# guy3540/Acoustic_Locating_VQ-VAE

Hardware: AMD Instinct MI355X
Metric: spectrograms/sec (train step), speech VQ-VAE default config (higher is better)
Workload: dtype x3mx_hb

## Files before the change

### acoustic_locating_vq-vae_amd/csrc/alvq_common.h

```cpp
#pragma once
#include <hip/hip_runtime.h>
#include <stdint.h>
#include <stdio.h>

#include "../../include/alvq.h"

namespace alvq {

void set_error(const char* fmt, ...);

enum Option { OPT_WIDE_MIN_TILES, OPT_FX_ROWS, OPT_FX_NARROW, OPT_FX_EPI, OPT_CONV_V2, OPT_CONV_K3, OPT_WGRAD_V3, OPT_VQ_REG, OPT_PHAT_LDS, OPT_COUNT };
long option(int id);

inline int check_launch(const char* what) {
  hipError_t e = hipGetLastError();
  if (e != hipSuccess) {
    set_error("%s: %s", what, hipGetErrorString(e));
    return (int)e;
  }
  return ALVQ_OK;
}

#define ALVQ_REQUIRE(cond, code, ...)  \
  do {                                 \
    if (!(cond)) {                     \
      alvq::set_error(__VA_ARGS__);    \
      return (code);                   \
    }                                  \
  } while (0)

struct DeviceOnce {
  bool done[64] = {};
  bool need() {
    int d = 0;
    if (hipGetDevice(&d) != hipSuccess || d < 0 || d >= 64) return true;
    if (done[d]) return false;
    done[d] = true;
    return true;
  }
};

constexpr int kWave = 64;
constexpr int kNumXcd = 8;

__device__ __forceinline__ int xcd_remap(int id, int n) {
  const int q = n / kNumXcd, r = n % kNumXcd;
  const int xcd = id % kNumXcd, local = id / kNumXcd;
  const int base = xcd < r ? xcd * (q + 1) : r * (q + 1) + (xcd - r) * q;
  return base + local;
}

typedef float f32x4 __attribute__((ext_vector_type(4)));
typedef float f32x16 __attribute__((ext_vector_type(16)));
typedef short bf16x8 __attribute__((ext_vector_type(8)));
typedef short bf16x4 __attribute__((ext_vector_type(4)));

int* fx_range_flag_ptr();
int* fx_range_sticky_ptr();

}

#include "block_reduce.h"
```

### acoustic_locating_vq-vae_amd/csrc/api.hip

```cpp
#include <stdarg.h>
#include <stdlib.h>
#include <string.h>

#include <atomic>

#include "alvq_common.h"

namespace alvq {
static thread_local char g_err[512] = "";
void set_error(const char* fmt, ...) {
  va_list ap;
  va_start(ap, fmt);
  vsnprintf(g_err, sizeof(g_err), fmt, ap);
  va_end(ap);
}

struct OptionSpec { const char* name; const char* env; long def; };
static const OptionSpec kSpecs[OPT_COUNT] = {
    {"wide_min_tiles", "ALVQ_WIDE_MIN_TILES", 192},
    {"fx_rows", "ALVQ_FX_ROWS", 0},
    {"fx_narrow", "ALVQ_FX_NARROW", 1},
    {"fx_epi", "ALVQ_FX_EPI", 1},
    {"conv_v2", "ALVQ_CONV_V2", 1},
    {"conv_k3", "ALVQ_CONV_K3", 1},
    {"wgrad_v3", "ALVQ_WGRAD_V3", 3},
    {"vq_reg", "ALVQ_VQ_REG", 1},
    {"phat_lds", "ALVQ_PHAT_LDS", 1},
};
static std::atomic<long> g_opt[OPT_COUNT];
static std::atomic<int> g_opt_ready{0};
static void options_init() {
  if (g_opt_ready.load(std::memory_order_acquire)) return;
  for (int i = 0; i < OPT_COUNT; ++i) {
    const char* e = getenv(kSpecs[i].env);
    g_opt[i].store(e ? atol(e) : kSpecs[i].def, std::memory_order_relaxed);
  }
  g_opt_ready.store(1, std::memory_order_release);
}
long option(int id) {
  options_init();
  return g_opt[id].load(std::memory_order_relaxed);
}
}

extern "C" const char* alvq_version(void) { return "alvq 0.4.0 (gfx950)"; }
extern "C" const char* alvq_last_error(void) { return alvq::g_err; }

extern "C" int alvq_set_option(const char* name, int64_t value) {
  ALVQ_REQUIRE(name, ALVQ_EINVAL, "alvq_set_option: null name");
  alvq::options_init();
  for (int i = 0; i < alvq::OPT_COUNT; ++i)
    if (!strcmp(name, alvq::kSpecs[i].name)) {
      alvq::g_opt[i].store((long)value, std::memory_order_relaxed);
      return ALVQ_OK;
    }
  alvq::set_error("alvq_set_option: unknown option '%s'", name);
  return ALVQ_EINVAL;
}

extern "C" int64_t alvq_get_option(const char* name) {
  if (name) {
    alvq::options_init();
    for (int i = 0; i < alvq::OPT_COUNT; ++i)
      if (!strcmp(name, alvq::kSpecs[i].name)) return alvq::g_opt[i].load(std::memory_order_relaxed);
  }
  alvq::set_error("alvq_get_option: unknown option '%s'", name ? name : "(null)");
  return INT64_MIN;
}
```

### acoustic_locating_vq-vae_amd/csrc/conv1d_bf16x3.hip

```cpp
#include <stdlib.h>

#include "alvq_common.h"
#include "bf16_common.h"
#include "conv_tile.h"
#include "nlc_host.h"
#include "wgrad_bias_reduce.h"
#include "wgrad_reduce.h"
#include "wgrad_tile.h"

namespace alvq {

struct ConvX3Args {
  ConvBArgs b;
  long x_plane, wp_plane, y_plane;
};

__device__ __forceinline__ void split2(float v, u16& hi, u16& lo) {
  hi = f2bf(v);
  lo = f2bf(v - bf2f(hi));
}

__device__ __forceinline__ void split_pack8(const float (&v)[8], u32x4& hi, u32x4& lo) {
#pragma unroll
  for (int e = 0; e < 4; ++e) {
    hi[e] = f2bf_pk(v[2 * e], v[2 * e + 1]);
    lo[e] = f2bf_pk(v[2 * e] - __uint_as_float(hi[e] << 16), v[2 * e + 1] - __uint_as_float(hi[e] & 0xffff0000u));
  }
}

template <int NNI>
__device__ __forceinline__ void wave_epilogue_x3(const ConvX3Args& ax, const f32x4 (&acc)[8][NNI], int m0, int r0, int li,
                                                 int kq, int wm0, int wn0) {
  const ConvBArgs& a = ax.b;
  const int Lp1 = a.L + 1, ndata = a.B * Lp1;
  const int mb0 = m0 + wm0 + (kq & 1) * 16 + (kq >> 1) * 8;
  const long pl = ax.y_plane;
#pragma unroll
  for (int ni = 0; ni < NNI; ++ni) {
    const int row = r0 + wn0 + ni * 16 + li;
    int b, l;
    const bool ok = row_valid(row, Lp1, ndata, &b, &l);
    const bool gaps = !__all(ok);
    const long o0 = (long)row * a.Mop + mb0;
    u16x8 s1h[4], s1l[4], mk[4];
#pragma unroll
    for (int mp = 0; mp < 8; mp += 2) {
      if (m0 + wm0 + mp * 16 >= a.Mop) continue;
      if (a.skip1) {
        s1h[mp / 2] = *(const u16x8*)(a.skip1 + o0 + mp * 16);
        s1l[mp / 2] = *(const u16x8*)(a.skip1 + pl + o0 + mp * 16);
      }
      if (a.mask) mk[mp / 2] = *(const u16x8*)(a.mask + o0 + mp * 16);
    }
    __builtin_amdgcn_sched_barrier(0);
#pragma unroll
    for (int mp = 0; mp < 8; mp += 2) {
      if (m0 + wm0 + mp * 16 >= a.Mop) continue;
      const long o = o0 + mp * 16;
      const int mb = mb0 + mp * 16;
      float v[8];
#pragma unroll
      for (int e = 0; e < 4; ++e) {
        const u32x2 r = __builtin_amdgcn_permlane16_swap(__float_as_uint(acc[mp][ni][e]), __float_as_uint(acc[mp + 1][ni][e]),
                                                         false, false);
        v[e] = __uint_as_float(r[0]);
        v[e + 4] = __uint_as_float(r[1]);
      }
      if (a.bias) {
        if (m0 + wm0 + mp * 16 + 32 <= a.M) {
          const f32x4 b0 = *(const f32x4*)(a.bias + mb), b1 = *(const f32x4*)(a.bias + mb + 4);
#pragma unroll
          for (int e = 0; e < 4; ++e) {
            v[e] += b0[e];
            v[4 + e] += b1[e];
          }
        } else {
#pragma unroll
          for (int e = 0; e < 8; ++e) v[e] += (mb + e < a.M) ? a.bias[mb + e] : 0.f;
        }
      }
      if (a.skip1) {
#pragma unroll
        for (int e = 0; e < 8; ++e) v[e] += bf2f(s1h[mp / 2][e]) + bf2f(s1l[mp / 2][e]);
      }
      if (a.skip2) {
        const u16x8 sh = *(const u16x8*)(a.skip2 + o), sl = *(const u16x8*)(a.skip2 + pl + o);
#pragma unroll
        for (int e = 0; e < 8; ++e) v[e] += bf2f(sh[e]) + bf2f(sl[e]);
      }
      if (a.relu & 1) {
#pragma unroll
        for (int e = 0; e < 8; ++e) v[e] = fmaxf(v[e], 0.f);
      }
      if (a.mask) {
#pragma unroll
        for (int e = 0; e < 8; ++e) v[e] = bf2f(mk[mp / 2][e]) > 0.f ? v[e] : 0.f;
      }
      u32x4 hi, lo;
      split_pack8(v, hi, lo);
      if (gaps) {
#pragma unroll
        for (int e = 0; e < 4; ++e) {
          hi[e] = ok ? hi[e] : 0u;
          lo[e] = ok ? lo[e] : 0u;
        }
      }
      *(u32x4*)(a.y + o) = hi;
      *(u32x4*)(a.y + pl + o) = lo;
      if (a.y2) {
        const u16x8 ph = *(const u16x8*)(a.post + o), pq = *(const u16x8*)(a.post + pl + o);
#pragma unroll
        for (int e = 0; e < 8; ++e) v[e] += bf2f(ph[e]) + bf2f(pq[e]);
        split_pack8(v, hi, lo);
        if (gaps) {
#pragma unroll
          for (int e = 0; e < 4; ++e) {
            hi[e] = ok ? hi[e] : 0u;
            lo[e] = ok ? lo[e] : 0u;
          }
        }
        *(u32x4*)(a.y2 + o) = hi;
        *(u32x4*)(a.y2 + pl + o) = lo;
      }
    }
  }
}

template <int NNI, int OPS>
__device__ __forceinline__ void wave_epilogue_x3_ordered(const ConvX3Args& ax, f32x4 (&acc)[8][NNI], int m0, int r0, int li,
                                                         int kq, int wm0, int wn0) {
  const ConvBArgs& a = ax.b;
  const int Lp1 = a.L + 1, ndata = a.B * Lp1;
  const int mb0 = m0 + wm0 + (kq & 1) * 16 + (kq >> 1) * 8;
  const long pl = ax.y_plane;
  const long o00 = (long)(r0 + wn0 + li) * a.Mop + mb0, oblk = (long)16 * a.Mop;
  u16x8 s1h[4], s1l[4];
  auto request = [&](int ni) {
#pragma unroll
    for (int p = 0; p < 4; ++p) {
      s1h[p] = *(const u16x8*)(a.skip1 + o00 + ni * oblk + p * 32);
      s1l[p] = *(const u16x8*)(a.skip1 + pl + o00 + ni * oblk + p * 32);
    }
  };
  if (OPS == 1) request(0);
  if (OPS == 2) {
#pragma unroll
    for (int mi = 0; mi < 8; ++mi) {
      const int c0 = m0 + wm0 + mi * 16 + kq * 4;
      f32x4 bv;
      if (m0 + wm0 + (mi & ~1) * 16 + 32 <= a.M) {
        bv = *(const f32x4*)(a.bias + c0);
      } else {
#pragma unroll
        for (int e = 0; e < 4; ++e) bv[e] = (c0 + e < a.M) ? a.bias[c0 + e] : 0.f;
      }
#pragma unroll
      for (int ni = 0; ni < NNI; ++ni)
#pragma unroll
        for (int e = 0; e < 4; ++e) acc[mi][ni][e] += bv[e];
    }
  }
  __builtin_amdgcn_sched_barrier(0);
#pragma unroll
  for (int ni = 0; ni < NNI; ++ni) {
    int b, l;
    const bool ok = row_valid(r0 + wn0 + ni * 16 + li, Lp1, ndata, &b, &l);
    const bool gaps = !__all(ok);
    u32x4 hi[4], lo[4];
#pragma unroll
    for (int p = 0; p < 4; ++p) {
      float v[8];
#pragma unroll
      for (int e = 0; e < 4; ++e) {
        const u32x2 r = __builtin_amdgcn_permlane16_swap(__float_as_uint(acc[2 * p][ni][e]), __float_as_uint(acc[2 * p + 1][ni][e]),
                                                         false, false);
        v[e] = __uint_as_float(r[0]);
        v[e + 4] = __uint_as_float(r[1]);
      }
      if (OPS == 1) {
#pragma unroll
        for (int e = 0; e < 8; ++e) v[e] += bf2f(s1h[p][e]) + bf2f(s1l[p][e]);
      }
      if (a.relu & 1) {
#pragma unroll
        for (int e = 0; e < 8; ++e) v[e] = fmaxf(v[e], 0.f);
      }
      split_pack8(v, hi[p], lo[p]);
      if (gaps) {
#pragma unroll
        for (int e = 0; e < 4; ++e) {
          hi[p][e] = ok ? hi[p][e] : 0u;
          lo[p][e] = ok ? lo[p][e] : 0u;
        }
      }
    }
    __builtin_amdgcn_sched_barrier(0);
    if (OPS == 1 && ni + 1 < NNI) request(ni + 1);
    __builtin_amdgcn_sched_barrier(0);
#pragma unroll
    for (int p = 0; p < 4; ++p) {
      *(u32x4*)(a.y + o00 + ni * oblk + p * 32) = hi[p];
      *(u32x4*)(a.y + pl + o00 + ni * oblk + p * 32) = lo[p];
    }
  }
}


template <int OUT, int KW, int NNI = 4>
__global__ __launch_bounds__(512, 2) void conv1d_bf16x3_kernel(ConvX3Args ax) {
  static_assert(NNI == 4 || NNI == 2 || NNI == 1, "4, 2 or 1 row fragments per wave");
  typedef ConvRings G;
  constexpr int MT = NNI == 4 ? G::M : 128;
  constexpr int RT = NNI == 1 ? 128 : G::R;
  const ConvBArgs& a = ax.b;
  extern __shared__ __attribute__((aligned(16))) unsigned char lds[];
  const int tid = threadIdx.x, lane = tid & 63;
  const int wave = __builtin_amdgcn_readfirstlane(tid >> 6);
  const int li = lane & 15, kq = lane >> 4;
  const int wm0 = NNI == 4 ? (wave >> 2) * 128 : 0, wn0 = NNI == 4 ? (wave & 3) * 64 : wave * 16 * NNI;

  const ConvTileOrigin o = conv_tile_origin<MT, RT>(a);
  const int m0 = o.m0, r0 = o.r0;
  const int Cp = a.Cp;
  const int srow = slab64_lane(lane).row;
  const unsigned lane_off = slab64_lane_off(lane, Cp);
  const long tap_w = (long)a.Mp128 * Cp * 2;
  const long row16 = (long)Cp * 32;
  const long wpl = ax.wp_plane * 2, xpl = ax.x_plane * 2;
  const char* const wb = (const char*)(a.wp + ((long)m0 + wave * 32) * Cp);
  const char* const xb = (const char*)(a.x + ((long)r0 - (KW - 1) / 2 + wave * 32) * Cp);
  const ConvRingStager<KW, MT, RT, false> st(wave, srow, lane_off, tap_w, row16, wpl, xpl, wb, xb);

  const int loffA = slab64_frag16(li, kq, 0);
  int loffB[KW];
#pragma unroll
  for (int t = 0; t < KW; ++t) loffB[t] = slab64_frag16(li, kq, t);
  const unsigned char* const abase = lds + wm0 * 64 + loffA;
  const unsigned char* const bbase = lds + G::XBASE + wn0 * 64;
  bf16x8_t fa0[8], fa1[8], fb0[NNI], fb1[NNI];
#define X3_RDA(DST, HALF, WS, PLANE)                                                               \
  {                                                                                                \
    const unsigned char* pa_ = abase + (WS) * G::WSTAGE + (PLANE) * G::SLAB;                       \
    _Pragma("unroll") for (int mi = (HALF) * 4; mi < (HALF) * 4 + 4; ++mi) DST[mi] = *(const bf16x8_t*)(pa_ + mi * 1024); \
  }
#define X3_RDB(DST, XS, TAP, PLANE)                                                                \
  {                                                                                                \
    const unsigned char* pb_ = bbase + (XS) * G::XSTAGE + (PLANE) * G::XSLAB + loffB[TAP];         \
    _Pragma("unroll") for (int ni = 0; ni < NNI; ++ni) DST[ni] = *(const bf16x8_t*)(pb_ + ni * 1024); \
  }

  f32x4 acc[8][NNI];
#pragma unroll
  for (int i = 0; i < 8; ++i)
#pragma unroll
    for (int j = 0; j < NNI; ++j) acc[i][j] = f32x4{0.f, 0.f, 0.f, 0.f};
#define X3_MM(A, B, HALF)                                                                          \
  _Pragma("unroll") for (int mi = (HALF) * 4; mi < (HALF) * 4 + 4; ++mi)                           \
  _Pragma("unroll") for (int ni = 0; ni < NNI; ++ni)                                               \
      asm("v_mfma_f32_16x16x32_bf16 %0, %1, %2, %0" : "+v"(acc[mi][ni]) : "v"(A[mi]), "v"(B[ni]));
#define X3_SB __builtin_amdgcn_sched_barrier(0);

  const int nch = Cp / G::K;
  const int n = nch * KW;
  const bool early = wave < 4;

  st.prologue(lds, n, nch);
  X3_RDA(fa0, 0, 0, 0)
  X3_RDA(fa0, 1, 0, 0)
  X3_RDB(fb0, 0, 0, 0)

#define X3_TILE(WS, XS, TAP, NWS, NXS, NTAP, BX, BY, DMA_)                                         \
  X3_MM(fa0, BX, 0) X3_SB X3_RDB(BY, XS, TAP, 1) X3_SB                                             \
  X3_MM(fa0, BX, 1) X3_SB X3_RDA(fa1, 0, WS, 1) X3_SB                                              \
  X3_MM(fa0, BY, 0) X3_SB X3_RDA(fa1, 1, WS, 1) X3_SB                                              \
  X3_MM(fa0, BY, 1) X3_SB                                                                          \
  asm volatile("s_waitcnt vmcnt(0) lgkmcnt(0)" ::: "memory");                                      \
  __builtin_amdgcn_s_barrier();                                                                    \
  if (early) { DMA_ }                                                                              \
  X3_MM(fa1, BX, 0) X3_SB X3_RDA(fa0, 0, NWS, 0) X3_RDB(BY, NXS, NTAP, 0) X3_SB                    \
  if (!early) { DMA_ }                                                                             \
  X3_MM(fa1, BX, 1) X3_SB X3_RDA(fa0, 1, NWS, 0) X3_SB

  if (KW == 3) {
    for (int c = 0; c < nch; c += 2) {
      const int t = 3 * c;
      X3_TILE(0, 0, 0, 1, 0, 1, fb0, fb1, if (t + 2 < n) st.issueW(lds, t + 2); if (c + 1 < nch) st.issueX(lds, c + 1, 0);)
      X3_TILE(1, 0, 1, 0, 0, 2, fb1, fb0, if (t + 3 < n) st.issueW(lds, t + 3); if (c + 1 < nch) st.issueX(lds, c + 1, 1);)
      X3_TILE(0, 0, 2, 1, 1, 0, fb0, fb1, if (t + 4 < n) st.issueW(lds, t + 4);)
      X3_TILE(1, 1, 0, 0, 1, 1, fb1, fb0, if (t + 5 < n) st.issueW(lds, t + 5); if (c + 2 < nch) st.issueX(lds, c + 2, 0);)
      X3_TILE(0, 1, 1, 1, 1, 2, fb0, fb1, if (t + 6 < n) st.issueW(lds, t + 6); if (c + 2 < nch) st.issueX(lds, c + 2, 1);)
      X3_TILE(1, 1, 2, 0, 0, 0, fb1, fb0, if (t + 7 < n) st.issueW(lds, t + 7);)
    }
  } else {
    for (int t = 0; t < n; t += 2) {
      X3_TILE(0, 0, 0, 1, 1, 0, fb0, fb1, if (t + 2 < n) { st.issueW(lds, t + 2); st.issueX(lds, t + 2, 0); st.issueX(lds, t + 2, 1); })
      X3_TILE(1, 1, 0, 0, 0, 0, fb1, fb0, if (t + 3 < n) { st.issueW(lds, t + 3); st.issueX(lds, t + 3, 0); st.issueX(lds, t + 3, 1); })
    }
  }
#undef X3_TILE
#undef X3_SB
#undef X3_MM
#undef X3_RDB
#undef X3_RDA
  asm volatile("s_nop 15\n\ts_nop 15" ::: "memory");

  if constexpr (OUT == 0) {
    const bool plain = !a.skip2 && !a.mask && !a.y2 && m0 + wm0 + 128 <= a.Mop;
    if (plain && a.skip1 && !a.bias) wave_epilogue_x3_ordered<NNI, 1>(ax, acc, m0, r0, li, kq, wm0, wn0);
    else if (plain && a.bias && !a.skip1) wave_epilogue_x3_ordered<NNI, 2>(ax, acc, m0, r0, li, kq, wm0, wn0);
    else wave_epilogue_x3(ax, acc, m0, r0, li, kq, wm0, wn0);
    return;
  }
  __syncthreads();
  conv_store_ncl<false, MT, RT>(a, lds, m0, r0, tid, nullptr, [&](float* Cs, int slab) {
    if ((wn0 >> 6) == slab) store_frags16<C_SLAB_STRIDE>(Cs, acc, li, kq, wm0, wn0 & 63);
  });
}

struct WgradX3Args {
  const u16* dy[WGRAD_MAXSEG];
  const u16* x[WGRAD_MAXSEG];
  int nseg;
  float* partial;
  float* bias_partial;
  long dy_plane, x_plane;
  int Mp, Cp, M, C;
  int mtiles, ctiles, splits, chunks_per_split, total_rows;
};

template <int KW, int NCF>
__global__ __launch_bounds__(512, 2) void conv1d_wgrad_bf16x3_kernel(WgradX3Args a) {
  constexpr int MT = 128, CT = 4 * NCF * 16;
  typedef WgradSlabs<KW, MT, CT, 2> Slabs;
  constexpr int YRB = Slabs::YRB, XRB = Slabs::XRB, YBYTES = Slabs::YBYTES, XBYTES = Slabs::XBYTES;
  extern __shared__ __attribute__((aligned(16))) unsigned char lds[];

  const int tid = threadIdx.x, lane = tid & 63;
  const int wave = __builtin_amdgcn_readfirstlane(tid >> 6);
  const int wm0 = (wave >> 2) * 64, wc0 = (wave & 3) * NCF * 16;
  const WgradWork w = wgrad_work<MT, CT>(a);
  const int n = w.n;
  WgradStager<WgradX3Args, KW, MT, CT, 2, LdsDmaAsm> st(a, wave, lane, w);

  int ybase, xbase[KW], yseg[4], xseg[NCF], xline[NCF];
  wgrad_frag16_bases<KW, NCF, YRB, XRB>(lane, wm0, wc0, ybase, xbase, yseg, xseg, xline);

  f32x4 acc[KW][4][NCF];
#pragma unroll
  for (int t = 0; t < KW; ++t)
#pragma unroll
    for (int i = 0; i < 4; ++i)
#pragma unroll
      for (int j = 0; j < NCF; ++j) acc[t][i][j] = f32x4{0.f, 0.f, 0.f, 0.f};
  const bool do_bias = a.bias_partial != nullptr && w.c0 == 0 && (wave & 3) == 0;
  f32x4 accb[4];
#pragma unroll
  for (int i = 0; i < 4; ++i) accb[i] = f32x4{0.f, 0.f, 0.f, 0.f};
  typedef short s16x8_t __attribute__((ext_vector_type(8)));
  const s16x8_t ones_raw = {0x3F80, 0x3F80, 0x3F80, 0x3F80, 0x3F80, 0x3F80, 0x3F80, 0x3F80};
  bf16x8_t ones = __builtin_bit_cast(bf16x8_t, ones_raw);
  asm volatile("" : "+v"(ones));

  bf16x8_t ah[4], al[4], b0[KW][NCF], b1[KW][NCF];
#define WX_RDA(DST, STAGE, PLANE, MI) \
  DST[MI] = wgrad_tr16_pair<bf16x8_t>(lds + ((STAGE) * STAGE_B + (PLANE) * YBYTES + (ybase ^ yseg[MI])), YRB);
#define WX_RDB(DST, STAGE, PLANE, TP, CF)                                                                                      \
  DST[TP][CF] = wgrad_tr16_pair<bf16x8_t>(                                                                                     \
      lds + ((STAGE) * STAGE_B + 2 * YBYTES + (PLANE) * XBYTES + ((xbase[TP] ^ xseg[CF]) + xline[CF])), XRB);
#define WX_MM(A, B, MI)                                                                                    \
  _Pragma("unroll") for (int tp = 0; tp < KW; ++tp)                                                        \
  _Pragma("unroll") for (int cf = 0; cf < NCF; ++cf)                                                       \
      asm("v_mfma_f32_16x16x32_bf16 %0, %1, %2, %0" : "+v"(acc[tp][MI][cf]) : "v"(A[MI]), "v"(B[tp][cf]));
#define WX_BIAS_ON(A, MI) asm("v_mfma_f32_16x16x32_bf16 %0, %1, %2, %0" : "+v"(accb[MI]) : "v"(A[MI]), "v"(ones));
#define WX_BIAS_OFF(A, MI)
#define WX_SB __builtin_amdgcn_sched_barrier(0);
  constexpr int STAGE_B = Slabs::STAGE;

#define WX_TILE(S, BX, BY, MORE, WX_BIAS)                                                                         \
                                                 \
  WX_MM(ah, BX, 0) WX_BIAS(ah, 0) WX_SB                                                                    \
  _Pragma("unroll") for (int tp = 0; tp < KW; ++tp) _Pragma("unroll") for (int cf = 0; cf < NCF; ++cf) WX_RDB(BY, S, 1, tp, cf) \
  WX_SB WX_MM(ah, BX, 1) WX_BIAS(ah, 1) WX_SB                                                              \
  WX_RDA(al, S, 1, 0) WX_RDA(al, S, 1, 1) WX_RDA(al, S, 1, 2) WX_RDA(al, S, 1, 3)                          \
  WX_SB WX_MM(ah, BX, 2) WX_BIAS(ah, 2) WX_MM(ah, BX, 3) WX_BIAS(ah, 3) WX_SB                              \
                                                                                       \
  WX_MM(ah, BY, 0) WX_MM(ah, BY, 1) WX_MM(ah, BY, 2) WX_MM(ah, BY, 3) WX_SB                                \
  asm volatile("s_waitcnt vmcnt(0) lgkmcnt(0)" ::: "memory");                                              \
  __builtin_amdgcn_s_barrier();                                                                            \
     \
  if (MORE) st.issue(lds, S);                                                                              \
  WX_MM(al, BX, 0) WX_BIAS(al, 0) WX_SB                                                                    \
  WX_RDA(ah, (S) ^ 1, 0, 0) WX_RDA(ah, (S) ^ 1, 0, 1) WX_RDA(ah, (S) ^ 1, 0, 2) WX_RDA(ah, (S) ^ 1, 0, 3)  \
  WX_SB WX_MM(al, BX, 1) WX_BIAS(al, 1) WX_SB                                                              \
  _Pragma("unroll") for (int tp = 0; tp < KW; ++tp) _Pragma("unroll") for (int cf = 0; cf < NCF; ++cf) WX_RDB(BY, (S) ^ 1, 0, tp, cf) \
  WX_SB WX_MM(al, BX, 2) WX_BIAS(al, 2) WX_MM(al, BX, 3) WX_BIAS(al, 3) WX_SB

  if (n > 0) {
    st.issue(lds, 0);
    if (n > 1) st.issue(lds, 1);
    st.wait_keep(n > 1 ? 1 : 0);
    __builtin_amdgcn_s_barrier();
    WX_RDA(ah, 0, 0, 0) WX_RDA(ah, 0, 0, 1) WX_RDA(ah, 0, 0, 2) WX_RDA(ah, 0, 0, 3)
#pragma unroll
    for (int tp = 0; tp < KW; ++tp)
#pragma unroll
      for (int cf = 0; cf < NCF; ++cf) WX_RDB(b0, 0, 0, tp, cf)
    if (do_bias) {
      for (int t = 0; t < n; t += 2) {
        WX_TILE(0, b0, b1, t + 2 < n, WX_BIAS_ON)
        WX_TILE(1, b1, b0, t + 3 < n, WX_BIAS_ON)
      }
    } else {
      for (int t = 0; t < n; t += 2) {
        WX_TILE(0, b0, b1, t + 2 < n, WX_BIAS_OFF)
        WX_TILE(1, b1, b0, t + 3 < n, WX_BIAS_OFF)
      }
    }
    asm volatile("s_nop 15\n\ts_nop 15" ::: "memory");
  }
#undef WX_TILE
#undef WX_SB
#undef WX_BIAS_ON
#undef WX_BIAS_OFF
#undef WX_MM
#undef WX_RDB
#undef WX_RDA

  wgrad_store16<KW, NCF>(a, w, lane, wm0, wc0, acc, do_bias, accb);
}

__global__ __launch_bounds__(256) void ncl_to_nlc_x3_kernel(const float* x, u16* y, long plane, int B, int C, int L, int Cp,
                                                            int rows_total) {
  __shared__ float tile[32][33];
  const int ct = Cp / 32;
  const int r0 = (blockIdx.x / ct) * 32, c0 = (blockIdx.x % ct) * 32;
  const int tx = threadIdx.x & 31, ty = threadIdx.x >> 5;
  const int Lp1 = L + 1, ndata = B * Lp1;
#pragma unroll
  for (int i = 0; i < 4; ++i) {
    const int c = c0 + ty + 8 * i, row = r0 + tx;
    int b, l;
    const bool ok = row_valid(row, Lp1, ndata, &b, &l) && c < C;
    tile[ty + 8 * i][tx] = ok ? x[((long)b * C + c) * L + l] : 0.f;
  }
  __syncthreads();
#pragma unroll
  for (int i = 0; i < 4; ++i) {
    const int row = r0 + ty + 8 * i, c = c0 + tx;
    if (row < rows_total) {
      u16 hi, lo;
      split2(tile[tx][ty + 8 * i], hi, lo);
      y[(long)row * Cp + c] = hi;
      y[plane + (long)row * Cp + c] = lo;
    }
  }
}

__global__ __launch_bounds__(256) void nlc_to_ncl_x3_kernel(const u16* x, long plane, float* y, int B, int C, int L, int Cp,
                                                            int rows_total) {
  __shared__ float tile[32][33];
  const int ct = Cp / 32;
  const int r0 = (blockIdx.x / ct) * 32, c0 = (blockIdx.x % ct) * 32;
  const int tx = threadIdx.x & 31, ty = threadIdx.x >> 5;
  const int Lp1 = L + 1, ndata = B * Lp1;
#pragma unroll
  for (int i = 0; i < 4; ++i) {
    const int row = r0 + ty + 8 * i, c = c0 + tx;
    tile[ty + 8 * i][tx] = row < rows_total ? bf2f(x[(long)row * Cp + c]) + bf2f(x[plane + (long)row * Cp + c]) : 0.f;
  }
  __syncthreads();
#pragma unroll
  for (int i = 0; i < 4; ++i) {
    const int c = c0 + ty + 8 * i, row = r0 + tx;
    int b, l;
    if (row_valid(row, Lp1, ndata, &b, &l) && c < C) y[((long)b * C + c) * L + l] = tile[tx][ty + 8 * i];
  }
}

__global__ __launch_bounds__(256) void relu_mask_x3_kernel(const u16* dy, const u16* t, u16* out, long plane8, long n8) {
  for (long e = (long)blockIdx.x * 256 + threadIdx.x; e < n8; e += (long)gridDim.x * 256) {
    const u16x8 dh = ((const u16x8*)dy)[e], dl = ((const u16x8*)dy)[plane8 + e], m = ((const u16x8*)t)[e];
    u16x8 oh, ol;
#pragma unroll
    for (int i = 0; i < 8; ++i) {
      const bool keep = bf2f(m[i]) > 0.f;
      oh[i] = keep ? dh[i] : (u16)0;
      ol[i] = keep ? dl[i] : (u16)0;
    }
    ((u16x8*)out)[e] = oh;
    ((u16x8*)out)[plane8 + e] = ol;
  }
}

template <int KW, int NCF>
static constexpr int wgrad_x3_lds() {
  return 2 * WgradSlabs<KW, 128, 4 * NCF * 16, 2>::STAGE;
}

static WgradTile wgrad_x3_tile(int KW) { return {128, KW == 3 ? 128 : 256}; }

constexpr int X3_BIAS_SPLITS = 64;

}

using namespace alvq;

extern "C" int64_t alvq_nlc_plane_bytes(int B, int L, int C) {
  return (B <= 0 || L <= 0 || C <= 0) ? -1 : nlc_plane_elems(B, L, C) * 2;
}

extern "C" int alvq_pack_weight_bf16x3(const float* w, void* wp, int M, int C, int KW, int w_layout, void* stream) {
  const alvq_pack_desc d{w, wp, M, C, KW, w_layout};
  return alvq_pack_weights_bf16_batch(&d, 1, 2, stream);
}

extern "C" int alvq_ncl_to_nlc_bf16x3(const float* x, void* y, int B, int C, int L, void* stream) {
  if (int rc = check_nlc_dims("alvq_ncl_to_nlc_bf16x3", x && y, B, C, L)) return rc;
  const NlcDims d(B, C, L);
  hipLaunchKernelGGL(ncl_to_nlc_x3_kernel, d.grid32(), dim3(256), 0, (hipStream_t)stream, x, (u16*)y, d.plane, B, C, L, d.Cp, d.rows);
  return check_launch("alvq_ncl_to_nlc_bf16x3");
}

extern "C" int alvq_nlc_to_ncl_bf16x3(const void* x, float* y, int B, int C, int L, void* stream) {
  if (int rc = check_nlc_dims("alvq_nlc_to_ncl_bf16x3", x && y, B, C, L)) return rc;
  const NlcDims d(B, C, L);
  hipLaunchKernelGGL(nlc_to_ncl_x3_kernel, d.grid32(), dim3(256), 0, (hipStream_t)stream, (const u16*)x, d.plane, y, B, C, L, d.Cp,
                     d.rows);
  return check_launch("alvq_nlc_to_ncl_bf16x3");
}

extern "C" int alvq_relu_mask_bf16x3(const void* dy, const void* t, void* out, int B, int C, int L, void* stream) {
  if (int rc = check_nlc_dims("alvq_relu_mask_bf16x3", dy && t && out, B, C, L)) return rc;
  const NlcDims d(B, C, L);
  const long n = (long)d.rows * d.Cp;
  long g = (n / 8 + 1023) / 1024;
  if (g > 2048) g = 2048;
  hipLaunchKernelGGL(relu_mask_x3_kernel, dim3((int)g), dim3(256), 0, (hipStream_t)stream, (const u16*)dy, (const u16*)t,
                     (u16*)out, d.plane / 8, n / 8);
  return check_launch("alvq_relu_mask_bf16x3");
}

static constexpr int x3_slot(int OUT, int KW, int NNI) { return ((NNI >> 1) * 2 + OUT) * 2 + (KW == 3); }
typedef KernelTable<void (*)(ConvX3Args), 12> X3Table;
static X3Table x3_table() {
  X3Table t;
  for_values<1, 2, 4>([&](auto nni) { for_values<0, 1>([&](auto out) { for_values<1, 3>([&](auto kw) {
    t.put(x3_slot(out, kw, nni), conv1d_bf16x3_kernel<out, kw, nni>, ConvRings::LDS);
  }); }); });
  return t;
}

extern "C" int alvq_conv1d_bf16x3(const void* x, const void* wp, const float* bias, const void* skip1, const void* skip2,
                                  const void* mask, const void* post, void* y, void* y2, float* y_ncl, int B, int C, int M,
                                  int L, int KW, int relu, void* stream) {
  if (int rc = check_conv_args("alvq_conv1d_bf16x3", x, wp, skip1, skip2, mask, post, y, y2, y_ncl, B, C, M, L, KW, relu, nullptr,
                               nullptr))
    return rc;
  const long rows = alvq_nlc_rows(B, L);
  ConvX3Args a{{(const u16*)x, (const u16*)wp, bias, (const u16*)skip1, (const u16*)skip2, (const u16*)mask, (const u16*)post,
                (u16*)y, (u16*)y2, y_ncl, B, L, pad_to(C, 64), M, pad_to(M, 64), pad_to(M, WP_ROWS), relu ? 1 : 0,
                (int)(rows / ConvRings::R), pad_to(M, ConvRings::M) / ConvRings::M},
               nlc_plane_elems(B, L, C), (long)alvq_packed_weight_elems(M, C, KW), nlc_plane_elems(B, L, M)};
  static const X3Table table = x3_table();
  static DeviceOnce attr;
  if (attr.need()) table.raise_lds_limit();
  const int forced = (int)option(OPT_FX_ROWS);
  const bool narrow = option(OPT_FX_NARROW) != 0 && (M <= 128 || (forced != 256 && a.b.rtiles * a.b.mtiles < 192) || forced == 128);
  if (narrow) a.b.mtiles = pad_to(M, 128) / 128;
  const bool small = narrow && forced != 256 && (a.b.rtiles * a.b.mtiles < 192 || forced == 128);
  if (small) a.b.rtiles = (int)(rows / 128);
  return table.launch(x3_slot(y ? 0 : 1, KW, small ? 1 : narrow ? 2 : 4), dim3(a.b.rtiles * a.b.mtiles), dim3(512),
                      (hipStream_t)stream, "alvq_conv1d_bf16x3", a);
}

extern "C" int64_t alvq_conv1d_wgrad_bf16x3_workspace_bytes(int B, int C, int M, int L, int KW) {
  return wgrad_workspace_bytes(B, C, M, L, KW, wgrad_x3_tile(KW), X3_BIAS_SPLITS);
}

extern "C" int alvq_conv1d_wgrad_bf16x3_splits(int B, int C, int M, int L, int KW, int nseg) {
  return wgrad_splits(B, C, M, L, KW, nseg, wgrad_x3_tile(KW));
}

static int wgrad_x3(const char* who, const void* const* dy, const void* const* x, int nseg, bool multi, float* dw, float* dbias,
                    void* workspace, int B, int C, int M, int L, int KW, int w_layout, int accumulate, hipStream_t s) {
  if (int rc = check_wgrad_args(who, dy, x, nseg, multi, dw, workspace, B, C, M, L, KW, w_layout, accumulate, false)) return rc;
  WgradX3Args a{};
  float* bpart;
  if (int rc = wgrad_plan("alvq_conv1d_wgrad_bf16x3", a, dy, x, nseg, workspace, B, C, M, L, KW, wgrad_x3_tile(KW), &bpart)) return rc;
  if (dbias) a.bias_partial = bpart;
  static const auto table = [] {
    KernelTable<void (*)(WgradX3Args), 2> t;
    for_values<1, 3>([&](auto kw) {
      constexpr int NCF = kw == 3 ? 2 : 4;
      t.put(kw == 3, conv1d_wgrad_bf16x3_kernel<kw, NCF>, wgrad_x3_lds<kw, NCF>());
    });
    return t;
  }();
  static DeviceOnce attr;
  if (attr.need()) table.raise_lds_limit();
  if (int rc = table.launch(KW == 3, dim3(a.mtiles * a.ctiles * a.splits), dim3(512), s, "alvq_conv1d_wgrad_bf16x3", a)) return rc;
  wgrad_reduce_launch((const float*)workspace, dw, a.splits, KW, M, C, w_layout, accumulate, s);
  if (dbias)
    hipLaunchKernelGGL(wgrad_bias_reduce_kernel, dim3((M + 255) / 256), dim3(256), 0, s, (const float*)bpart, dbias, a.splits,
                       a.Mp, M, accumulate, (const float*)nullptr);
  return check_launch("alvq_conv1d_wgrad_bf16x3/reduce");
}

extern "C" int alvq_conv1d_wgrad_bf16x3(const void* dy, const void* x, float* dw, float* dbias, void* workspace, int B, int C,
                                        int M, int L, int KW, int w_layout, int accumulate, void* stream) {
  return wgrad_x3("alvq_conv1d_wgrad_bf16x3", &dy, &x, 1, false, dw, dbias, workspace, B, C, M, L, KW, w_layout, accumulate,
                  (hipStream_t)stream);
}

extern "C" int alvq_conv1d_wgrad_bf16x3_multi(const void* const* dy, const void* const* x, int nseg, float* dw, void* workspace,
                                              int B, int C, int M, int L, int KW, int w_layout, int accumulate, void* stream) {
  return wgrad_x3("alvq_conv1d_wgrad_bf16x3_multi", dy, x, nseg, true, dw, nullptr, workspace, B, C, M, L, KW, w_layout, accumulate,
                  (hipStream_t)stream);
}
```

### acoustic_locating_vq-vae_amd/csrc/conv_tile.h

```cpp
#pragma once
#include "alvq_common.h"
#include "bf16_common.h"

namespace alvq {

struct ConvTileOrigin {
  int m0, r0;
};
template <int MT, int RT>
__device__ __forceinline__ ConvTileOrigin conv_tile_origin(const ConvBArgs& a) {
  const int tile = xcd_remap(blockIdx.x, a.mtiles * a.rtiles);
  return {(tile % a.mtiles) * MT, (tile / a.mtiles) * RT};
}

enum SlabKey { SLAB_KEY_ROWS, SLAB_KEY_TAPS };
template <SlabKey KEY = SLAB_KEY_ROWS>
__device__ __forceinline__ int slab64_key(int quad) {
  return KEY == SLAB_KEY_TAPS ? (quad & 1) * 2 : (quad == 0 ? 0 : 4 - quad);
}

struct Slab64Lane {
  int row, grp;
};
template <SlabKey KEY = SLAB_KEY_ROWS>
__device__ __forceinline__ Slab64Lane slab64_lane(int lane) {
  const int key = slab64_key<KEY>((lane >> 4) & 3);
  return {lane >> 2, (lane & 3) ^ key};
}
template <SlabKey KEY = SLAB_KEY_ROWS>
__device__ __forceinline__ unsigned slab64_lane_off(int lane, int Cp) {
  const Slab64Lane s = slab64_lane<KEY>(lane);
  return (unsigned)(s.row * Cp + s.grp * 8) * 2u;
}

template <SlabKey KEY = SLAB_KEY_ROWS>
__device__ __forceinline__ int slab64_frag16(int li, int kq, int t) {
  const int r = li + t;
  return r * 64 + ((kq ^ slab64_key<KEY>((r >> 2) & 3)) << 4);
}
__device__ __forceinline__ int slab64_frag32(int r32, int g, int t) {
  const int r = r32 + t, key = slab64_key((r >> 2) & 3);
  return r * 64 + ((g ^ key) << 4);
}

__device__ __forceinline__ void lds_dma16(const char* sbase, unsigned lds_dst, unsigned lane_off) {
  asm volatile("s_mov_b32 m0, %2\n\ts_nop 0\n\tglobal_load_lds_dwordx4 %0, %1" ::"v"(lane_off), "s"(sbase), "s"(lds_dst)
               : "memory");
}
__device__ __forceinline__ unsigned lds_addr(const unsigned char* lds) {
  return (unsigned)(unsigned long)((const __attribute__((address_space(3))) unsigned char*)lds);
}
struct LdsDmaBuiltin {
  static __device__ __forceinline__ void copy(const u16* base, long elem, unsigned char* lds, int stage, int off) {
    unsigned char* const dst = lds + stage;
    glds16(base + elem, dst + off);
  }
};
struct LdsDmaAsm {
  static __device__ __forceinline__ void copy(const u16* base, long elem, unsigned char* lds, int stage, int off) {
    const unsigned dst = lds_addr(lds) + stage + off;
    lds_dma16((const char*)base, dst, (unsigned)(elem * 2));
  }
};

constexpr int V2_M = 256, V2_R = 256, V2_K = 32;
constexpr int V2_HALF = V2_M * V2_K * 2;
constexpr int C_SLAB_STRIDE = V2_M + 4;
constexpr int C_SLAB_BYTES = 64 * C_SLAB_STRIDE * 4;

struct ConvRings {
  static constexpr int M = 256, R = 256, K = 32;
  static constexpr int SLAB = M * K * 2;
  static constexpr int WSTAGE = 2 * SLAB;
  static constexpr int XSLAB = 272 * 64;
  static constexpr int XSTAGE = 2 * XSLAB;
  static constexpr int XBASE = 2 * WSTAGE;
  static constexpr int LDS = XBASE + 2 * XSTAGE;
  static_assert(C_SLAB_BYTES <= LDS, "C slab must fit");
};

template <int KW, int MT, int RT, bool PIECEWISE>
struct ConvRingStager {
  typedef ConvRings G;
  const int &wave, &srow;
  const unsigned& lane_off;
  const long &tap_w, &row16, &wpl, &xpl;
  const char *const &wb, *const &xb;
  __device__ __forceinline__ ConvRingStager(const int& wave_, const int& srow_, const unsigned& lane_off_, const long& tap_w_,
                                            const long& row16_, const long& wpl_, const long& xpl_, const char* const& wb_,
                                            const char* const& xb_)
      : wave(wave_), srow(srow_), lane_off(lane_off_), tap_w(tap_w_), row16(row16_), wpl(wpl_), xpl(xpl_), wb(wb_), xb(xb_) {}
  __device__ __forceinline__ void pieceW(unsigned char* lds, int t, int k) const { pieceW_<true>(lds, t, k); }
  __device__ __forceinline__ void pieceX(unsigned char* lds, int chunk, int plane, int k) const { pieceX_<true>(lds, chunk, plane, k); }
  __device__ __forceinline__ void issueW(unsigned char* lds, int t) const {
    if constexpr (!PIECEWISE)
      if (wave * 32 >= MT) return;
    pieceW_<PIECEWISE>(lds, t, 0);
    pieceW_<PIECEWISE>(lds, t, 1);
    pieceW_<PIECEWISE>(lds, t, 2);
    pieceW_<PIECEWISE>(lds, t, 3);
  }
  __device__ __forceinline__ void issueX(unsigned char* lds, int chunk, int plane) const {
    if constexpr (!PIECEWISE)
      if (wave * 32 >= RT) return;
    pieceX_<PIECEWISE>(lds, chunk, plane, 0);
    pieceX_<PIECEWISE>(lds, chunk, plane, 1);
    pieceX_<PIECEWISE>(lds, chunk, plane, 2);
  }
  __device__ __forceinline__ void prologue(unsigned char* lds, int n, int nch) const {
    issueX(lds, 0, 0);
    issueX(lds, 0, 1);
    issueW(lds, 0);
    if (n > 1) issueW(lds, 1);
    if (KW == 1 && nch > 1) {
      issueX(lds, 1, 0);
      issueX(lds, 1, 1);
    }
    asm volatile("s_waitcnt vmcnt(0)" ::: "memory");
    __builtin_amdgcn_s_barrier();
  }
 private:
  template <bool GUARDED>
  __device__ __forceinline__ void pieceW_(unsigned char* lds, int t, int k) const {
    if constexpr (GUARDED)
      if (wave * 32 >= MT) return;
    const int chunk = t / KW, tap = t - chunk * KW;
    const unsigned dst = lds_addr(lds) + (t & 1) * G::WSTAGE + wave * 2048 + (k >> 1) * G::SLAB + (k & 1) * 1024;
    lds_dma16(wb + tap * tap_w + chunk * (G::K * 2) + (k >> 1) * wpl + (k & 1) * row16, dst, lane_off);
  }
  template <bool GUARDED>
  __device__ __forceinline__ void pieceX_(unsigned char* lds, int chunk, int plane, int k) const {
    const unsigned dst = lds_addr(lds) + G::XBASE + (chunk & 1) * G::XSTAGE + plane * G::XSLAB + wave * 2048;
    const char* xs = xb + plane * xpl + chunk * (G::K * 2);
    if constexpr (GUARDED)
      if (wave * 32 >= RT) return;
    if (k < 2) lds_dma16(xs + k * row16, dst + k * 1024, lane_off);
    else if (KW == 3 && wave == RT / 32 - 1 && srow < 2) lds_dma16(xs + 2 * row16, dst + 2048, lane_off);
  }
};

template <bool SCALED, int MT, int RT, class Write>
__device__ __forceinline__ void conv_store_ncl(const ConvBArgs& a, unsigned char* lds, int m0, int r0, int tid,
                                               const float* out_scale, Write write) {
  float oscale = 1.f;
  if constexpr (SCALED) oscale = out_scale ? *out_scale : 1.f;
  float* Cs = (float*)lds;
  for (int slab = 0; slab < RT / 64; ++slab) {
    write(Cs, slab);
    __syncthreads();
    const int Lp1 = a.L + 1, ndata = a.B * Lp1;
    const int rl = tid & 63, row = r0 + slab * 64 + rl;
    int b, l;
    if (row_valid(row, Lp1, ndata, &b, &l)) {
      for (int ml = tid >> 6; ml < MT; ml += 8) {
        const int m = m0 + ml;
        if (m >= a.M) break;
        const float v = Cs[rl * C_SLAB_STRIDE + ml] + (a.bias ? a.bias[m] : 0.f);
        a.y_ncl[((long)b * a.M + m) * a.L + l] = SCALED ? v * oscale : v;
      }
    }
    __syncthreads();
  }
}

template <int CSTRIDE, int NMI, int NNI>
__device__ __forceinline__ void store_frags16(float* Cs, const f32x4 (&acc)[NMI][NNI], int li, int kq, int wm0, int rl0) {
#pragma unroll
  for (int mi = 0; mi < NMI; ++mi)
#pragma unroll
    for (int ni = 0; ni < NNI; ++ni) {
      const int rl = rl0 + ni * 16 + li, ml = wm0 + mi * 16 + kq * 4;
      *(f32x4*)(Cs + rl * CSTRIDE + ml) = acc[mi][ni];
    }
}

struct FragSet {
  bf16x8_t a[8];
  bf16x8_t b[4];
};

template <int NMI, int NNI, int F16 = 0>
__device__ __forceinline__ void wave_epilogue_bf16(const ConvBArgs& a, const f32x4 (&acc)[NMI][NNI], int m0, int r0, int li,
                                                   int kq, int wm0, int wn0);

template <int NMI, int NNI, int F16, bool S1, bool S2, bool BITS>
__device__ __forceinline__ void wave_epilogue_dgrad16(const ConvBArgs& a, const f32x4 (&acc)[NMI][NNI], int m0, int r0, int li,
                                                      int kq, int wm0, int wn0);

template <int OUT, int F16 = 0>
__device__ __forceinline__ void tile256_epilogue(const ConvBArgs& a, const f32x4 (&acc)[8][4], unsigned char* lds, int m0,
                                                 int r0, int wave, int tid, int li, int kq, int wm0) {
  if (OUT == 0) {
    const int wn0 = (wave & 3) * 64;
    const bool dgrad = (a.mask_bits || a.mask) && !a.bias && !a.y2 && !a.bits_out && !(a.relu & 1) && (a.skip1 || !a.skip2) &&
                       m0 + wm0 + 128 <= a.Mop;
    if (!dgrad) wave_epilogue_bf16<8, 4, F16>(a, acc, m0, r0, li, kq, wm0, wn0);
    else if (a.mask_bits) {
      if (a.skip2) wave_epilogue_dgrad16<8, 4, F16, true, true, true>(a, acc, m0, r0, li, kq, wm0, wn0);
      else if (a.skip1) wave_epilogue_dgrad16<8, 4, F16, true, false, true>(a, acc, m0, r0, li, kq, wm0, wn0);
      else wave_epilogue_dgrad16<8, 4, F16, false, false, true>(a, acc, m0, r0, li, kq, wm0, wn0);
    } else {
      if (a.skip2) wave_epilogue_dgrad16<8, 4, F16, true, true, false>(a, acc, m0, r0, li, kq, wm0, wn0);
      else if (a.skip1) wave_epilogue_dgrad16<8, 4, F16, true, false, false>(a, acc, m0, r0, li, kq, wm0, wn0);
      else wave_epilogue_dgrad16<8, 4, F16, false, false, false>(a, acc, m0, r0, li, kq, wm0, wn0);
    }
    return;
  }
  conv_store_ncl<true, V2_M, V2_R>(a, lds, m0, r0, tid, a.out_scale, [&](float* Cs, int slab) {
    if ((wave & 3) == slab) store_frags16<C_SLAB_STRIDE>(Cs, acc, li, kq, wm0, 0);
  });
}

template <int NMI, int NNI, int F16>
__device__ __forceinline__ void wave_epilogue_bf16(const ConvBArgs& a, const f32x4 (&acc)[NMI][NNI], int m0, int r0, int li,
                                                   int kq, int wm0, int wn0) {
  static_assert(NMI % 2 == 0, "fragments are swapped in pairs");
  elem_saturate<F16>();
  unsigned watch = 0;
  const int Lp1 = a.L + 1, ndata = a.B * Lp1;
  const int mb0 = m0 + wm0 + (kq & 1) * 16 + (kq >> 1) * 8;
#pragma unroll
  for (int ni = 0; ni < NNI; ++ni) {
    const int row = r0 + wn0 + ni * 16 + li;
    int b, l;
    const bool ok = row_valid(row, Lp1, ndata, &b, &l);
    const bool gaps = !__all(ok);
    const long o0 = (long)row * a.Mop + mb0;
    u16x8 s1[NMI / 2], s2[NMI / 2], mk[NMI / 2];
#pragma unroll
    for (int mp = 0; mp < NMI; mp += 2) {
      if (m0 + wm0 + mp * 16 >= a.Mop) continue;
      if (a.skip1) s1[mp / 2] = *(const u16x8*)(a.skip1 + o0 + mp * 16);
      if (a.skip2) s2[mp / 2] = *(const u16x8*)(a.skip2 + o0 + mp * 16);
      if (a.mask && !a.mask_bits) mk[mp / 2] = *(const u16x8*)(a.mask + o0 + mp * 16);
    }
    __builtin_amdgcn_sched_barrier(0);
#pragma unroll
    for (int mp = 0; mp < NMI; mp += 2) {
      if (m0 + wm0 + mp * 16 >= a.Mop) continue;
      const long o = o0 + mp * 16;
      const int mb = mb0 + mp * 16;
      float v[8];
#pragma unroll
      for (int e = 0; e < 4; ++e) {
        const u32x2 r = __builtin_amdgcn_permlane16_swap(__float_as_uint(acc[mp][ni][e]), __float_as_uint(acc[mp + 1][ni][e]),
                                                         false, false);
        v[e] = __uint_as_float(r[0]);
        v[e + 4] = __uint_as_float(r[1]);
      }
      if (a.bias) {
        if (m0 + wm0 + mp * 16 + 32 <= a.M) {
          const f32x4 b0 = *(const f32x4*)(a.bias + mb), b1 = *(const f32x4*)(a.bias + mb + 4);
#pragma unroll
          for (int e = 0; e < 4; ++e) {
            v[e] += b0[e];
            v[4 + e] += b1[e];
          }
        } else {
#pragma unroll
          for (int e = 0; e < 8; ++e) v[e] += (mb + e < a.M) ? a.bias[mb + e] : 0.f;
        }
      }
      if (a.skip1) {
#pragma unroll
        for (int e = 0; e < 8; ++e) v[e] += elem2f<F16>(s1[mp / 2][e]);
      }
      if (a.skip2) {
#pragma unroll
        for (int e = 0; e < 8; ++e) v[e] += elem2f<F16>(s2[mp / 2][e]);
      }
      if (a.relu & 1) {
#pragma unroll
        for (int e = 0; e < 8; ++e) v[e] = fmaxf(v[e], 0.f);
      }
      if (a.mask_bits) {
        const int bt = (int)a.mask_bits[o >> 3];
#pragma unroll
        for (int e = 0; e < 8; ++e) v[e] = __uint_as_float(__float_as_uint(v[e]) & (unsigned)((bt << (31 - e)) >> 31));
      } else if (a.mask) {
#pragma unroll
        for (int e = 0; e < 8; ++e) v[e] = (short)mk[mp / 2][e] > 0 ? v[e] : 0.f;
      }
      u32x4 out;
#pragma unroll
      for (int e = 0; e < 4; ++e) out[e] = elem_pk<F16>(v[2 * e], v[2 * e + 1]);
      if (gaps) {
#pragma unroll
        for (int e = 0; e < 4; ++e) out[e] = ok ? out[e] : 0u;
      }
      *(u32x4*)(a.y + o) = out;
// ... 120 lines not shown
```

Before: 7653.

## Add specialized bf16x3 conv epilogues, fused post-residual output, and tap-keyed X slab layout

Adds compile-time epilogue variants (EPI 1-4) to the bf16x3 conv kernel, selected on the host by which of bias, skip and post operands are present. The EPI 4 variant fuses the skip1 residual, ReLU and post addition into one pass that writes both y and y2 without going through the generic epilogue. The X staging also switches to a tap-keyed LDS slab layout for KW=3, using a separate lane offset and fragment addressing. The kernel table grows to hold the extra instantiations, which adds code size, and the new layout carries a risk of bank conflicts or addressing mistakes.

```diff
diff --git a/acoustic_locating_vq-vae_amd/csrc/alvq_common.h b/acoustic_locating_vq-vae_amd/csrc/alvq_common.h
--- a/acoustic_locating_vq-vae_amd/csrc/alvq_common.h
+++ b/acoustic_locating_vq-vae_amd/csrc/alvq_common.h
@@ -9,7 +9,7 @@
 
 void set_error(const char* fmt, ...);
 
-enum Option { OPT_WIDE_MIN_TILES, OPT_FX_ROWS, OPT_FX_NARROW, OPT_FX_EPI, OPT_CONV_V2, OPT_CONV_K3, OPT_WGRAD_V3, OPT_VQ_REG, OPT_PHAT_LDS, OPT_COUNT };
+enum Option { OPT_WIDE_MIN_TILES, OPT_FX_ROWS, OPT_FX_NARROW, OPT_FX_EPI, OPT_X3_EPI, OPT_CONV_V2, OPT_CONV_K3, OPT_WGRAD_V3, OPT_VQ_REG, OPT_PHAT_LDS, OPT_COUNT };
 long option(int id);
 
 inline int check_launch(const char* what) {
diff --git a/acoustic_locating_vq-vae_amd/csrc/api.hip b/acoustic_locating_vq-vae_amd/csrc/api.hip
--- a/acoustic_locating_vq-vae_amd/csrc/api.hip
+++ b/acoustic_locating_vq-vae_amd/csrc/api.hip
@@ -21,6 +21,7 @@
     {"fx_rows", "ALVQ_FX_ROWS", 0},
     {"fx_narrow", "ALVQ_FX_NARROW", 1},
     {"fx_epi", "ALVQ_FX_EPI", 1},
+    {"x3_epi", "ALVQ_X3_EPI", 1},
     {"conv_v2", "ALVQ_CONV_V2", 1},
     {"conv_k3", "ALVQ_CONV_K3", 1},
     {"wgrad_v3", "ALVQ_WGRAD_V3", 3},
diff --git a/acoustic_locating_vq-vae_amd/csrc/conv1d_bf16x3.hip b/acoustic_locating_vq-vae_amd/csrc/conv1d_bf16x3.hip
--- a/acoustic_locating_vq-vae_amd/csrc/conv1d_bf16x3.hip
+++ b/acoustic_locating_vq-vae_amd/csrc/conv1d_bf16x3.hip
@@ -126,7 +126,7 @@
   }
 }
 
-template <int NNI, int OPS>
+template <int NNI, int OPS, bool PIN = false>
 __device__ __forceinline__ void wave_epilogue_x3_ordered(const ConvX3Args& ax, f32x4 (&acc)[8][NNI], int m0, int r0, int li,
                                                          int kq, int wm0, int wn0) {
   const ConvBArgs& a = ax.b;
@@ -143,6 +143,7 @@
     }
   };
   if (OPS == 1) request(0);
+  if (OPS == 1 && PIN) asm volatile("" ::: "memory");
   if (OPS == 2) {
 #pragma unroll
     for (int mi = 0; mi < 8; ++mi) {
@@ -205,10 +206,84 @@
   }
 }
 
-
-template <int OUT, int KW, int NNI = 4>
+template <int NNI>
+__device__ __forceinline__ void wave_epilogue_x3_post(const ConvX3Args& ax, f32x4 (&acc)[8][NNI], int m0, int r0, int li, int kq,
+                                                      int wm0, int wn0) {
+  const ConvBArgs& a = ax.b;
+  const int Lp1 = a.L + 1, ndata = a.B * Lp1;
+  const int mb0 = m0 + wm0 + (kq & 1) * 16 + (kq >> 1) * 8;
+  const long pl = ax.y_plane;
+  const long o00 = (long)(r0 + wn0 + li) * a.Mop + mb0, oblk = (long)16 * a.Mop;
+  u16x8 s1h[4], s1l[4], psh[4], psl[4];
+  auto request = [&](int ni) {
+#pragma unroll
+    for (int p = 0; p < 4; ++p) {
+      s1h[p] = *(const u16x8*)(a.skip1 + o00 + ni * oblk + p * 32);
+      s1l[p] = *(const u16x8*)(a.skip1 + pl + o00 + ni * oblk + p * 32);
+    }
+#pragma unroll
+    for (int p = 0; p < 4; ++p) {
+      psh[p] = *(const u16x8*)(a.post + o00 + ni * oblk + p * 32);
+      psl[p] = *(const u16x8*)(a.post + pl + o00 + ni * oblk + p * 32);
+    }
+  };
+  request(0);
+  asm volatile("" ::: "memory");
+  __builtin_amdgcn_sched_barrier(0);
+#pragma unroll
+  for (int ni = 0; ni < NNI; ++ni) {
+    int b, l;
+    const bool ok = row_valid(r0 + wn0 + ni * 16 + li, Lp1, ndata, &b, &l);
+    const bool gaps = !__all(ok);
+    u32x4 hi[4], lo[4], hi2[4], lo2[4];
+#pragma unroll
+    for (int p = 0; p < 4; ++p) {
+      float v[8];
+#pragma unroll
+      for (int e = 0; e < 4; ++e) {
+        const u32x2 r = __builtin_amdgcn_permlane16_swap(__float_as_uint(acc[2 * p][ni][e]), __float_as_uint(acc[2 * p + 1][ni][e]),
+                                                         false, false);
+        v[e] = __uint_as_float(r[0]);
+        v[e + 4] = __uint_as_float(r[1]);
+      }
+#pragma unroll
+      for (int e = 0; e < 8; ++e) v[e] += bf2f(s1h[p][e]) + bf2f(s1l[p][e]);
+      if (a.relu & 1) {
+#pragma unroll
+        for (int e = 0; e < 8; ++e) v[e] = fmaxf(v[e], 0.f);
+      }
+      split_pack8(v, hi[p], lo[p]);
+#pragma unroll
+      for (int e = 0; e < 8; ++e) v[e] += bf2f(psh[p][e]) + bf2f(psl[p][e]);
+      split_pack8(v, hi2[p], lo2[p]);
+      if (gaps) {
+#pragma unroll
+        for (int e = 0; e < 4; ++e) {
+          hi[p][e] = ok ? hi[p][e] : 0u;
+          lo[p][e] = ok ? lo[p][e] : 0u;
+          hi2[p][e] = ok ? hi2[p][e] : 0u;
+          lo2[p][e] = ok ? lo2[p][e] : 0u;
+        }
+      }
+    }
+    __builtin_amdgcn_sched_barrier(0);
+    if (ni + 1 < NNI) request(ni + 1);
+    __builtin_amdgcn_sched_barrier(0);
+#pragma unroll
+    for (int p = 0; p < 4; ++p) {
+      *(u32x4*)(a.y + o00 + ni * oblk + p * 32) = hi[p];
+      *(u32x4*)(a.y + pl + o00 + ni * oblk + p * 32) = lo[p];
+      *(u32x4*)(a.y2 + o00 + ni * oblk + p * 32) = hi2[p];
+      *(u32x4*)(a.y2 + pl + o00 + ni * oblk + p * 32) = lo2[p];
+    }
+  }
+}
+
+
+template <int OUT, int KW, int NNI = 4, int EPI = 0>
 __global__ __launch_bounds__(512, 2) void conv1d_bf16x3_kernel(ConvX3Args ax) {
   static_assert(NNI == 4 || NNI == 2 || NNI == 1, "4, 2 or 1 row fragments per wave");
+  static_assert(EPI == 0 || (OUT == 0 && NNI != 1 && EPI <= 4), "operand sets: bf16x3 output, 256- and 128-channel tiles");
   typedef ConvRings G;
   constexpr int MT = NNI == 4 ? G::M : 128;
   constexpr int RT = NNI == 1 ? 128 : G::R;
@@ -222,19 +297,21 @@
   const ConvTileOrigin o = conv_tile_origin<MT, RT>(a);
   const int m0 = o.m0, r0 = o.r0;
   const int Cp = a.Cp;
+  constexpr SlabKey XKEY = KW == 3 ? SLAB_KEY_TAPS : SLAB_KEY_ROWS;
   const int srow = slab64_lane(lane).row;
   const unsigned lane_off = slab64_lane_off(lane, Cp);
+  const unsigned lane_off_x = slab64_lane_off<XKEY>(lane, Cp);
   const long tap_w = (long)a.Mp128 * Cp * 2;
   const long row16 = (long)Cp * 32;
   const long wpl = ax.wp_plane * 2, xpl = ax.x_plane * 2;
   const char* const wb = (const char*)(a.wp + ((long)m0 + wave * 32) * Cp);
   const char* const xb = (const char*)(a.x + ((long)r0 - (KW - 1) / 2 + wave * 32) * Cp);
-  const ConvRingStager<KW, MT, RT, false> st(wave, srow, lane_off, tap_w, row16, wpl, xpl, wb, xb);
+  const ConvRingStager<KW, MT, RT, false> st(wave, srow, lane_off, lane_off_x, tap_w, row16, wpl, xpl, wb, xb);
 
   const int loffA = slab64_frag16(li, kq, 0);
   int loffB[KW];
 #pragma unroll
-  for (int t = 0; t < KW; ++t) loffB[t] = slab64_frag16(li, kq, t);
+  for (int t = 0; t < KW; ++t) loffB[t] = slab64_frag16<XKEY>(li, kq, t);
   const unsigned char* const abase = lds + wm0 * 64 + loffA;
   const unsigned char* const bbase = lds + G::XBASE + wn0 * 64;
   bf16x8_t fa0[8], fa1[8], fb0[NNI], fb1[NNI];
@@ -304,17 +381,25 @@
 #undef X3_RDA
   asm volatile("s_nop 15\n\ts_nop 15" ::: "memory");
 
-  if constexpr (OUT == 0) {
+  if constexpr (EPI == 1) {
+    wave_epilogue_x3_ordered<NNI, 0>(ax, acc, m0, r0, li, kq, wm0, wn0);
+  } else if constexpr (EPI == 2) {
+    wave_epilogue_x3_ordered<NNI, 2>(ax, acc, m0, r0, li, kq, wm0, wn0);
+  } else if constexpr (EPI == 3) {
+    wave_epilogue_x3_ordered<NNI, 1, true>(ax, acc, m0, r0, li, kq, wm0, wn0);
+  } else if constexpr (EPI == 4) {
+    wave_epilogue_x3_post<NNI>(ax, acc, m0, r0, li, kq, wm0, wn0);
+  } else if constexpr (OUT == 0) {
     const bool plain = !a.skip2 && !a.mask && !a.y2 && m0 + wm0 + 128 <= a.Mop;
     if (plain && a.skip1 && !a.bias) wave_epilogue_x3_ordered<NNI, 1>(ax, acc, m0, r0, li, kq, wm0, wn0);
     else if (plain && a.bias && !a.skip1) wave_epilogue_x3_ordered<NNI, 2>(ax, acc, m0, r0, li, kq, wm0, wn0);
     else wave_epilogue_x3(ax, acc, m0, r0, li, kq, wm0, wn0);
-    return;
-  }
-  __syncthreads();
-  conv_store_ncl<false, MT, RT>(a, lds, m0, r0, tid, nullptr, [&](float* Cs, int slab) {
-    if ((wn0 >> 6) == slab) store_frags16<C_SLAB_STRIDE>(Cs, acc, li, kq, wm0, wn0 & 63);
-  });
+  } else {
+    __syncthreads();
+    conv_store_ncl<false, MT, RT>(a, lds, m0, r0, tid, nullptr, [&](float* Cs, int slab) {
+      if ((wn0 >> 6) == slab) store_frags16<C_SLAB_STRIDE>(Cs, acc, li, kq, wm0, wn0 & 63);
+    });
+  }
 }
 
 struct WgradX3Args {
@@ -540,12 +625,17 @@
   return check_launch("alvq_relu_mask_bf16x3");
 }
 
-static constexpr int x3_slot(int OUT, int KW, int NNI) { return ((NNI >> 1) * 2 + OUT) * 2 + (KW == 3); }
-typedef KernelTable<void (*)(ConvX3Args), 12> X3Table;
+static constexpr int x3_slot(int OUT, int KW, int NNI, int EPI = 0) {
+  return EPI == 0 ? ((NNI >> 1) * 2 + OUT) * 2 + (KW == 3) : 12 + (((NNI >> 2) * 2 + (KW == 3)) * 4 + EPI - 1);
+}
+typedef KernelTable<void (*)(ConvX3Args), 28> X3Table;
 static X3Table x3_table() {
   X3Table t;
   for_values<1, 2, 4>([&](auto nni) { for_values<0, 1>([&](auto out) { for_values<1, 3>([&](auto kw) {
     t.put(x3_slot(out, kw, nni), conv1d_bf16x3_kernel<out, kw, nni>, ConvRings::LDS);
+  }); }); });
+  for_values<2, 4>([&](auto nni) { for_values<1, 3>([&](auto kw) { for_values<1, 2, 3, 4>([&](auto epi) {
+    t.put(x3_slot(0, kw, nni, epi), conv1d_bf16x3_kernel<0, kw, nni, epi>, ConvRings::LDS);
   }); }); });
   return t;
 }
@@ -569,7 +659,12 @@
   if (narrow) a.b.mtiles = pad_to(M, 128) / 128;
   const bool small = narrow && forced != 256 && (a.b.rtiles * a.b.mtiles < 192 || forced == 128);
   if (small) a.b.rtiles = (int)(rows / 128);
-  return table.launch(x3_slot(y ? 0 : 1, KW, small ? 1 : narrow ? 2 : 4), dim3(a.b.rtiles * a.b.mtiles), dim3(512),
+  int epi = 0;
+  if (y && !small && !skip2 && !mask && a.b.Mop % (narrow ? 128 : ConvRings::M) == 0 && option(OPT_X3_EPI) != 0) {
+    if (!post) epi = bias ? (skip1 ? 0 : 2) : (skip1 ? 3 : 1);
+    else if (skip1 && !bias) epi = 4;
+  }
+  return table.launch(x3_slot(y ? 0 : 1, KW, small ? 1 : narrow ? 2 : 4, epi), dim3(a.b.rtiles * a.b.mtiles), dim3(512),
                       (hipStream_t)stream, "alvq_conv1d_bf16x3", a);
 }
 
diff --git a/acoustic_locating_vq-vae_amd/csrc/conv_tile.h b/acoustic_locating_vq-vae_amd/csrc/conv_tile.h
--- a/acoustic_locating_vq-vae_amd/csrc/conv_tile.h
+++ b/acoustic_locating_vq-vae_amd/csrc/conv_tile.h
@@ -83,13 +83,19 @@
 struct ConvRingStager {
   typedef ConvRings G;
   const int &wave, &srow;
-  const unsigned& lane_off;
+  const unsigned &lane_off, &lane_off_x;
   const long &tap_w, &row16, &wpl, &xpl;
   const char *const &wb, *const &xb;
   __device__ __forceinline__ ConvRingStager(const int& wave_, const int& srow_, const unsigned& lane_off_, const long& tap_w_,
                                             const long& row16_, const long& wpl_, const long& xpl_, const char* const& wb_,
                                             const char* const& xb_)
-      : wave(wave_), srow(srow_), lane_off(lane_off_), tap_w(tap_w_), row16(row16_), wpl(wpl_), xpl(xpl_), wb(wb_), xb(xb_) {}
+      : wave(wave_), srow(srow_), lane_off(lane_off_), lane_off_x(lane_off_), tap_w(tap_w_), row16(row16_), wpl(wpl_), xpl(xpl_),
+        wb(wb_), xb(xb_) {}
+  __device__ __forceinline__ ConvRingStager(const int& wave_, const int& srow_, const unsigned& lane_off_, const unsigned& lane_off_x_,
+                                            const long& tap_w_, const long& row16_, const long& wpl_, const long& xpl_,
+                                            const char* const& wb_, const char* const& xb_)
+      : wave(wave_), srow(srow_), lane_off(lane_off_), lane_off_x(lane_off_x_), tap_w(tap_w_), row16(row16_), wpl(wpl_), xpl(xpl_),
+        wb(wb_), xb(xb_) {}
   __device__ __forceinline__ void pieceW(unsigned char* lds, int t, int k) const { pieceW_<true>(lds, t, k); }
   __device__ __forceinline__ void pieceX(unsigned char* lds, int chunk, int plane, int k) const { pieceX_<true>(lds, chunk, plane, k); }
   __device__ __forceinline__ void issueW(unsigned char* lds, int t) const {
@@ -134,8 +140,8 @@
     const char* xs = xb + plane * xpl + chunk * (G::K * 2);
     if constexpr (GUARDED)
       if (wave * 32 >= RT) return;
-    if (k < 2) lds_dma16(xs + k * row16, dst + k * 1024, lane_off);
-    else if (KW == 3 && wave == RT / 32 - 1 && srow < 2) lds_dma16(xs + 2 * row16, dst + 2048, lane_off);
+    if (k < 2) lds_dma16(xs + k * row16, dst + k * 1024, lane_off_x);
+    else if (KW == 3 && wave == RT / 32 - 1 && srow < 2) lds_dma16(xs + 2 * row16, dst + 2048, lane_off_x);
   }
 };
 
```

After: 7700 (median of 6 runs). No clear change (+0.6%).
